# OpenGVLab/VisionLLM

Hardware: NVIDIA H100
Metric: img_text_pairs_per_sec_fwd_1024px_256tok (higher is better)
Workload: dtype bf16

## Files before the change

### include/vllm_b200.h

```cpp
#ifndef VLLM_B200_H
#define VLLM_B200_H
#include <stdint.h>
#include <stddef.h>
#ifdef __cplusplus
extern "C" {
#endif

#define VLLM_OK 0
#define VLLM_EINVAL (-1)
#define VLLM_EUNSUPPORTED (-2)
#define VLLM_EALIGN (-3)

const char* vllm_version(void);

#define VLLM_MSDA_STRICT 1
int vllm_msda_forward_f32(const float* value, const int64_t* spatial_shapes, const int64_t* level_start_index,
                          const float* sampling_loc, const float* attn_weight, float* out, int batch,
                          int spatial_size, int num_heads, int channels, int num_levels, int num_query,
                          int num_point, const int64_t* host_shapes_hint, int flags, void* stream);
int vllm_msda_forward_bf16v(const void* value, const int64_t* spatial_shapes, const int64_t* level_start_index,
                            const float* sampling_loc, const float* attn_weight, void* out, int out_bf16, int batch,
                            int spatial_size, int num_heads, int channels, int num_levels, int num_query,
                            int num_point, const int64_t* host_shapes_hint, void* stream);
int vllm_msda_forward_f64(const double* value, const int64_t* spatial_shapes, const int64_t* level_start_index,
// ... 4 lines not shown
                           const float* sampling_loc, const float* attn_weight, const float* grad_output,
                           float* grad_value, float* grad_sampling_loc, float* grad_attn_weight, int batch,
                           int spatial_size, int num_heads, int channels, int num_levels, int num_query,
                           int num_point, void* stream);
int vllm_msda_backward_f64(const double* value, const int64_t* spatial_shapes, const int64_t* level_start_index,
                           const double* sampling_loc, const double* attn_weight, const double* grad_output,
                           double* grad_value, double* grad_sampling_loc, double* grad_attn_weight, int batch,
                           int spatial_size, int num_heads, int channels, int num_levels, int num_query,
                           int num_point, void* stream);
int vllm_msda_sample_indices_f32(const int64_t* spatial_shapes, const float* sampling_loc, int32_t* out_hwm,
                                 long long n_samples, int num_levels, int num_point, void* stream);
#define VLLM_MSDA_DEFAULT 0
#define VLLM_MSDA_NO_HINT 4
#define VLLM_MSDA_BF16_NO_WINDOW 32
#define VLLM_MSDA_FP32_WINDOW 33
int vllm_msda_set_variant(int variant);
int vllm_msda_set_window(int patch_h, int patch_w, int halo0);
int vllm_msda_set_window_fill(int tma);
int vllm_msda_forward_fused_bf16(const void* value, const int64_t* level_start_index, const void* qp, int ld_qp,
                                 const float* reference_points, void* out, int out_bf16, void* attn_weights_out, int batch,
                                 int spatial_size, int num_heads, int channels, int num_levels, int num_query, int num_point,
                                 const int64_t* host_shapes_hint, void* stream);

int vllm_dcnv3_forward_f32(const float* input, const float* offset, const float* mask, float* out, int N,
                           int H_in, int W_in, int H_out, int W_out, int group, int group_channels,
                           int kernel_h, int kernel_w, int stride_h, int stride_w, int pad_h, int pad_w,
                           int dilation_h, int dilation_w, float offset_scale, int flags, void* stream);

int vllm_dcnv3_backward_f32(const float* input, const float* offset, const float* mask, const float* grad_output,
                            float* grad_input, float* grad_offset, float* grad_mask, int N, int H_in, int W_in,
                            int H_out, int W_out, int group, int group_channels, int kernel_h, int kernel_w,
                            int stride_h, int stride_w, int pad_h, int pad_w, int dilation_h, int dilation_w,
                            float offset_scale, void* stream);

#define VLLM_ACT_NONE 0
#define VLLM_ACT_GELU 1
#define VLLM_ACT_RELU 2
#define VLLM_ACT_SILU 3
#define VLLM_ACT_SWIGLU 4
#define VLLM_ACT_QUICKGELU 5
int vllm_gemm_bf16(const void* A, int lda, const void* B, int ldb, void* C, int ldc, int M, int N, int K,
                   const void* bias, const void* colscale, const void* residual, int ldr, int act, int out_f32,
                   void* stream);
int vllm_gemm_bf16_rowmask(const void* A, int lda, const void* B, int ldb, void* C, int ldc, int M, int N, int K,
                           const void* bias, const void* colscale, const void* residual, int ldr, int act, int out_f32,
                           const unsigned char* row_keep, void* stream);
int vllm_gemm_set_sm_limit(int all_gemms, int scatter_gemm);
int vllm_conv_rows_bf16(const void* xpad, long long pad_pixels, int channels, int padded_width, int kernel_h,
                        int kernel_w, const void* weight, int ldw, void* out, int ldo, int out_channels,
                        const void* bias, int act, void* stream);
#define VLLM_GEMM_DEFAULT 0
#define VLLM_GEMM_WIDE_TILE 2
#define VLLM_GEMM_NARROW_TILE 3
int vllm_gemm_set_variant(int variant);

int vllm_rmsnorm_bf16(const void* x, long long ldx, const void* weight, void* y, long long ldy, long long rows,
                      int cols, float eps, void* stream);
int vllm_layernorm_bf16(const void* x, long long ldx, const void* weight, const void* bias, void* y, long long ldy,
                        long long rows, int cols, float eps, void* stream);
int vllm_layernorm_gelu_bf16(const void* x, long long ldx, const void* weight, const void* bias, void* y,
                             long long ldy, long long rows, int cols, float eps, void* stream);
int vllm_layernorm_gather_bf16(const void* x, long long ldx, const int64_t* index, long long rows_in, long long rows_out,
                               long long batch, const void* weight, const void* bias, void* y, long long ldy, int cols,
                               float eps, void* stream);
int vllm_layernorm_residual_bf16(const void* x, long long ldx, const void* weight, const void* bias,
                                 const void* residual, long long ldr, void* y, long long ldy, long long rows, int cols,
                                 float eps, void* stream);
int vllm_dcnv3_prep_f32(const void* packed, long long ld, void* offset, void* mask, void* scale, long long rows,
                        int group, int taps, void* stream);
int vllm_dcnv3_blend_bf16(const void* core, const void* xproj, const void* scale, void* out, long long rows,
                          int channels, int group_channels, void* stream);
int vllm_dwconv_nhwc_bf16(const void* x, const void* weight_taps, const void* bias, void* y, int batch, int height,
                          int width, int channels, int kernel, void* stream);
long long vllm_groupnorm_workspace_bytes(int batch, int groups);
int vllm_groupnorm_nhwc_bf16_grid(const void* x, void* y, const void* gamma, const void* beta, int batch, long long h, long long w,
                                  long long x_w_pitch, long long x_image_pitch, int channels, int groups, float eps, int relu,
                                  void* workspace, long long workspace_bytes, void* stream);
int vllm_upsample_add_nhwc_bf16_ex(const void* top, long long top_image_pitch, const void* lateral, void* out, int batch, int in_h,
                                   int in_w, int out_h, int out_w, int channels, int out_pad, void* stream);
int vllm_rope_bf16(void* x, long long ld, const void* cos, const void* sin, long long tokens, int heads,
                   int head_dim, void* stream);

int vllm_attention_bf16(const void* q, const void* k, const void* v, void* o, int batch, int Tq, int Tk,
                        int heads, int kv_heads, int head_dim, long long q_batch_pitch,
                        long long q_token_pitch, long long k_batch_pitch, long long k_token_pitch,
                        long long v_batch_pitch, long long v_token_pitch, long long o_batch_pitch,
                        long long o_token_pitch, const int* seqlens, const unsigned char* key_mask,
                        const unsigned char* attn_mask, const float* attn_bias, int bias_batches, int causal,
                        float scale, void* workspace, long long workspace_bytes, void* stream);
int vllm_attention_mask_tiles(const unsigned char* attn_mask, long long n_batch_heads, int Tq, int Tk, int* tile_counts,
                              int* tile_lists, void* stream);
int vllm_attention_bf16_tiles(const void* q, const void* k, const void* v, void* o, int batch, int Tq, int Tk,
                              int heads, int kv_heads, int head_dim, long long q_batch_pitch,
                              long long q_token_pitch, long long k_batch_pitch, long long k_token_pitch,
                              long long v_batch_pitch, long long v_token_pitch, long long o_batch_pitch,
                              long long o_token_pitch, const int* seqlens, const unsigned char* key_mask,
                              const unsigned char* attn_mask, float scale, const int* tile_counts,
                              const int* tile_lists, void* stream);
#define VLLM_ATTN_DEFAULT 0
#define VLLM_ATTN_WARP_MMA 1
int vllm_attention_set_variant(int variant);
int vllm_attention_set_splits(int n);

int vllm_peer_alloc(void** ptr, size_t bytes);
int vllm_peer_free(void* ptr);
int vllm_peer_handle_bytes(void);
// ... 69 lines not shown
```

### visionllm_b200/_lib.py

```python
import contextlib
import ctypes
import os
import threading

_HERE = os.path.dirname(os.path.abspath(__file__))
LIB_PATH = os.path.join(_HERE, "lib", "libvllm_b200.so")

_lock = threading.Lock()
_lib = None
_launches = 0

c_i64p = ctypes.POINTER(ctypes.c_int64)
vp = ctypes.c_void_p
ci = ctypes.c_int
cll = ctypes.c_longlong
cf = ctypes.c_float

_SIGNATURES = {
    "vllm_version": (ctypes.c_char_p, []),
    "vllm_msda_forward_f32": (ci, [vp, vp, vp, vp, vp, vp, ci, ci, ci, ci, ci, ci, ci, vp, ci, vp]),
    "vllm_msda_forward_bf16v": (ci, [vp, vp, vp, vp, vp, vp, ci, ci, ci, ci, ci, ci, ci, ci, vp, vp]),
    "vllm_msda_forward_f64": (ci, [vp, vp, vp, vp, vp, vp, ci, ci, ci, ci, ci, ci, ci, vp]),
    "vllm_msda_backward_f32": (ci, [vp] * 9 + [ci] * 7 + [vp]),
    "vllm_msda_backward_f64": (ci, [vp] * 9 + [ci] * 7 + [vp]),
# ... 14 lines not shown
    "vllm_dcnv3_backward_f32": (ci, [vp] * 7 + [ci] * 15 + [cf, vp]),
    "vllm_gemm_set_sm_limit": (ci, [ci, ci]),
    "vllm_gemm_bf16": (ci, [vp, ci, vp, ci, vp, ci, ci, ci, ci, vp, vp, vp, ci, ci, ci, vp]),
    "vllm_gemm_bf16_rowmask": (ci, [vp, ci, vp, ci, vp, ci, ci, ci, ci, vp, vp, vp, ci, ci, ci, vp, vp]),
    "vllm_conv_rows_bf16": (ci, [vp, cll, ci, ci, ci, ci, vp, ci, vp, ci, ci, vp, ci, vp]),
    "vllm_gemm_bf16_tn": (ci, [vp, ci, ci, vp, ci, ci, vp, ci, ci, ci, ci, ci, vp]),
    "vllm_gemm_bf16_batched": (ci, [vp, ci, ci, vp, ci, ci, vp, ci, ci, ci, ci, ci, ci, ci, vp]),
    "vllm_gemm_bf16_batched_grouped": (ci, [vp, ci, ci, vp, ci, ci, vp, ci, ci, ci, ci, ci, ci, ci, ci, ci, vp]),
    "vllm_head_stack_bf16": (ci, [vp, vp, ci, ci, ci, ci, ci, ci, vp]),
    "vllm_head_stack_qkv_bf16": (ci, [vp, cll, vp, vp, vp, ci, ci, ci, ci, ci, ci, vp]),
    "vllm_rmsnorm_bwd_partials": (ci, [cll]),
    "vllm_rmsnorm_bwd_ws_bf16": (ci, [vp, cll, vp, vp, cll, vp, cll, vp, vp, ci, cll, ci, cf, vp]),
    "vllm_swiglu_fwd_bf16": (ci, [vp, cll, vp, cll, cll, ci, vp]),
    "vllm_swiglu_bwd_bf16": (ci, [vp, cll, vp, cll, vp, cll, cll, ci, vp]),
    "vllm_softmax_causal_bf16": (ci, [vp, cll, cll, ci, cf, vp]),
    "vllm_attn_ds_bf16": (ci, [vp, vp, cll, cll, ci, cf, vp]),
    "vllm_ce_loss_f32": (ci, [vp, cll, vp, vp, cll, ci, vp, vp, cll, vp]),
    "vllm_scale_rows_bf16": (ci, [vp, cll, cll, ci, vp, vp]),
    "vllm_gemm_set_variant": (ci, [ci]),
    "vllm_rmsnorm_bf16": (ci, [vp, cll, vp, vp, cll, cll, ci, cf, vp]),
    "vllm_layernorm_bf16": (ci, [vp, cll, vp, vp, vp, cll, cll, ci, cf, vp]),
    "vllm_layernorm_gelu_bf16": (ci, [vp, cll, vp, vp, vp, cll, cll, ci, cf, vp]),
    "vllm_layernorm_gather_bf16": (ci, [vp, cll, vp, cll, cll, cll, vp, vp, vp, cll, ci, cf, vp]),
    "vllm_layernorm_residual_bf16": (ci, [vp, cll, vp, vp, vp, cll, vp, cll, cll, ci, cf, vp]),
    "vllm_dcnv3_prep_f32": (ci, [vp, cll, vp, vp, vp, cll, ci, ci, vp]),
    "vllm_dcnv3_blend_bf16": (ci, [vp, vp, vp, vp, cll, ci, ci, vp]),
    "vllm_dwconv_nhwc_bf16": (ci, [vp, vp, vp, vp, ci, ci, ci, ci, ci, vp]),
    "vllm_rope_bf16": (ci, [vp, cll, vp, vp, cll, ci, ci, vp]),
    "vllm_groupnorm_workspace_bytes": (cll, [ci, ci]),
    "vllm_upsample_add_nhwc_bf16_ex": (ci, [vp, cll, vp, vp, ci, ci, ci, ci, ci, ci, ci, vp]),
    "vllm_groupnorm_nhwc_bf16_grid": (ci, [vp, vp, vp, vp, ci, cll, cll, cll, cll, ci, ci, cf, ci, vp, cll, vp]),
    "vllm_attention_bf16": (ci, [vp, vp, vp, vp, ci, ci, ci, ci, ci, ci, cll, cll, cll, cll, cll, cll, cll, cll,
                                 vp, vp, vp, vp, ci, ci, cf, vp, cll, vp]),
    "vllm_attention_bf16_tiles": (ci, [vp, vp, vp, vp, ci, ci, ci, ci, ci, ci, cll, cll, cll, cll, cll, cll, cll, cll,
                                       vp, vp, vp, cf, vp, vp, vp]),
    "vllm_attention_mask_tiles": (ci, [vp, cll, ci, ci, vp, vp, vp]),
    "vllm_attention_set_variant": (ci, [ci]),
    "vllm_attention_set_splits": (ci, [ci]),
    "vllm_peer_alloc": (ci, [ctypes.POINTER(vp), ctypes.c_size_t]),
    "vllm_peer_free": (ci, [vp]),
    "vllm_peer_handle_bytes": (ci, []),
    "vllm_peer_export": (ci, [vp, vp]),
    "vllm_peer_open": (ci, [vp, ctypes.POINTER(vp)]),
    "vllm_peer_close": (ci, [vp]),
    "vllm_gemm_bf16_scatter": (ci, [vp, ci, vp, ci, vp, vp, ci, ci, ci, ci, ci, vp]),
    "vllm_tp_reduce_norm_bf16": (ci, [vp, ci, cll, vp, vp, cf, vp, ci, cll, vp, ctypes.c_uint, vp, ci, ci, ci, vp]),
    "vllm_tp_norm_ctas": (ci, [ci]),
    "vllm_tp_wait": (ci, [vp, ctypes.c_uint, vp]),
    "vllm_tp_signal": (ci, [vp, ci, ctypes.c_uint, vp]),
}


MSDA_DEFAULT, MSDA_NO_HINT, MSDA_BF16_NO_WINDOW, MSDA_FP32_WINDOW = 0, 4, 32, 33
GEMM_DEFAULT, GEMM_WIDE_TILE, GEMM_NARROW_TILE = 0, 2, 3
ATTN_DEFAULT, ATTN_WARP_MMA = 0, 1

_KNOB_DEFAULTS = {"msda_set_variant": (MSDA_DEFAULT,), "msda_set_window": (0, 0, 0), "msda_set_window_fill": (-1,),
                  "gemm_set_variant": (GEMM_DEFAULT,), "gemm_set_sm_limit": (0, 0), "attention_set_variant": (ATTN_DEFAULT,),
                  "attention_set_splits": (0,)}


class VllmB200Error(RuntimeError):
    pass


def exported_symbols():
    return sorted(_SIGNATURES)


def lib():
    global _lib
    if _lib is None:
        with _lock:
            if _lib is None:
                if not os.path.exists(LIB_PATH):
                    raise ImportError(
                        f"{LIB_PATH} is missing: build it with `make` or "
                        "`python -c 'import __graft_entry__ as g; g.build()'`. "
                        "visionllm_b200 has no CPU/eager fallback.")
                L = ctypes.CDLL(LIB_PATH)
                for name, (res, args) in _SIGNATURES.items():
                    fn = getattr(L, name)
                    fn.restype = res
                    fn.argtypes = args
                _lib = L
    return _lib


_ERR = {-1: "invalid argument", -2: "unsupported shape", -3: "misaligned pointer"}


def check(rc, what):
    global _launches
    _launches += 1
    if rc == 0:
        return
    if rc < 0:
        raise VllmB200Error(f"{what}: {_ERR.get(rc, 'error')} (rc={rc})")
    raise VllmB200Error(f"{what}: CUDA error {rc} at launch")


@contextlib.contextmanager
def knob(name, *values):
    fn = getattr(lib(), "vllm_" + name)
    rc = fn(*values)
    if rc != 0:
        raise VllmB200Error(f"vllm_{name}{values}: {_ERR.get(rc, 'error')} (rc={rc})")
# ... 14 lines not shown
```

### visionllm_b200/csrc/gemm.cu

```cuda
#include "common.cuh"
#include "tc_common.cuh"
#include "vllm_b200.h"

namespace {

constexpr int BM = 128, BK = 64, THREADS = 384, CONSUMER_WARPS = 8, CONSUMER_THREADS = CONSUMER_WARPS * 32;
constexpr int A_BYTES = BM * BK * 2;
constexpr int EPI_BUF = 16 * 128;
constexpr int SMEM_LIMIT = 232448;

enum { ACT_NONE = 0, ACT_GELU = 1, ACT_RELU = 2, ACT_SILU = 3, ACT_SWIGLU = 4, ACT_QUICKGELU = 5 };

struct GemmArgs {
  int M, N, K;
  void* C; int ldc;
  const __nv_bfloat16* bias; const __nv_bfloat16* colscale; const __nv_bfloat16* residual; int ldr;
  int act; int out_f32;
  const unsigned char* row_keep;
  int tiles_m, tiles_n;
  int group_m;
  int a_seg_kb, a_seg_rows;
  int sc_rows;
  void* sc_dst[8];
  uint32_t* sc_flag[8];
  int a_mn, b_mn;
  int bt_rows, causal;
  int group, reduce;
};

struct TilePlan { int skip, kb0, kb1, segs, b_row_off, a_k_off, b_k_off; };
__device__ __forceinline__ TilePlan plan_tile(const GemmArgs& g, int m0, int n0, int rows_per_tile, int num_kb) {
  TilePlan p{0, 0, num_kb, 1, 0, 0, 0};
  if (g.bt_rows) {
    const int bh = m0 / g.bt_rows, ml = m0 - bh * g.bt_rows;
    const int a_mat = g.reduce ? bh * g.group : bh;
    const int b_mat = g.reduce ? bh * g.group : bh / g.group;
    p.segs = g.reduce ? g.group : 1;
    p.b_row_off = b_mat * g.N;
    p.a_k_off = a_mat * g.K;
    p.b_k_off = b_mat * g.K;
    if (g.causal == 1 && n0 >= ml + rows_per_tile) p.skip = 1;
    if (g.causal == 2) p.kb0 = ml / BK;
    if (g.causal == 3) { const int e = (ml + rows_per_tile + BK - 1) / BK; p.kb1 = e < num_kb ? e : num_kb; }
  }
  return p;
}

template <int BN> struct Cfg {
  static constexpr int B_BYTES = BN * BK * 2;
  static constexpr int STAGE_BYTES = A_BYTES + B_BYTES;
  static constexpr int STAGES = BN == 256 ? 4 : 6;
  static constexpr int EPI_OFF = STAGES * STAGE_BYTES;
  static constexpr int BAR_OFF = EPI_OFF + CONSUMER_WARPS * 2 * EPI_BUF;
  static constexpr int BIAS_OFF = BAR_OFF + 256;
  static constexpr int SCALE_OFF = BIAS_OFF + 2 * BN + 4;
  static constexpr int KEEP_OFF = SCALE_OFF + 2 * BN + 4;
  static constexpr int SMEM = 1024  + KEEP_OFF + BM + 4;
  static_assert(8 * (2 * STAGES + 2 * CONSUMER_WARPS) <= 256, "mbarriers overflow their slot");
  static_assert(SMEM <= SMEM_LIMIT, "shared memory over the per-block limit");
};

__device__ __forceinline__ float gelu_erf(float x) { return 0.5f * x * (1.f + erff(x * 0.70710678118654752f)); }
__device__ __forceinline__ float silu(float x) { return x / (1.f + __expf(-x)); }

__device__ __forceinline__ void tile_coords(int t, int tiles_m, int tiles_n, int group_m, int& tm, int& tn) {
  const int per_group = group_m * tiles_n;
  const int group = t / per_group;
  const int first = group * group_m;
  const int gsz = min(group_m, tiles_m - first);
  const int in = t - group * per_group;
  tm = first + in % gsz;
  tn = in / gsz;
}

template <int BN, int TA, int TB>
__device__ __forceinline__ void mma_kblock(float (&acc)[BN / 2], uint32_t sa, uint32_t sb, bool first_kb) {
  const uint64_t adesc = TA ? tc::wgmma_desc_sw128(sa, 8192, 1024) : tc::wgmma_desc_sw128(sa, 16, 1024);
  const uint64_t bdesc = TB ? tc::wgmma_desc_sw128(sb, 8192, 1024) : tc::wgmma_desc_sw128(sb, 16, 1024);
  constexpr uint64_t astep = TA ? 128 : 2, bstep = TB ? 128 : 2;
#pragma unroll
  for (int k = 0; k < BK / 16; ++k) {
    if constexpr (BN == 256)
      tc::wgmma_m64n256k16_ss<TA, TB>(acc, adesc + astep * k, bdesc + bstep * k, !(first_kb && k == 0));
    else
      tc::wgmma_m64n128k16_ss<TA, TB>(acc, adesc + astep * k, bdesc + bstep * k, !(first_kb && k == 0));
  }
}

enum { EPI_BF16 = 0, EPI_SWIGLU = 1, EPI_F32 = 2, EPI_SCATTER = 3 };

__device__ __forceinline__ int swz(int r, int b) { return r * 128 + ((((b >> 4) ^ r) & 7) << 4) + (b & 15); }

template <int BN, int TA, int TB, int EPI>
__global__ void __launch_bounds__(THREADS, 1)
gemm_bf16_wgmma_kernel(const __grid_constant__ CUtensorMap tmap_a, const __grid_constant__ CUtensorMap tmap_b,
                       const __grid_constant__ CUtensorMap tmap_c, const __grid_constant__ CUtensorMap tmap_r,
                       const GemmArgs g) {
  using C_ = Cfg<BN>;
  constexpr int STAGES = C_::STAGES;
  extern __shared__ uint8_t smem_raw[];
  const uint32_t smem_base = (tc::smem_u32(smem_raw) + 1023u) & ~1023u;
  uint8_t* smem_gen = smem_raw + (smem_base - tc::smem_u32(smem_raw));
  const uint32_t bar_base = smem_base + C_::BAR_OFF;
  auto full_bar = [&](int s) { return bar_base + 8 * s; };
  auto empty_bar = [&](int s) { return bar_base + 8 * (STAGES + s); };
  auto res_bar = [&](int i) { return bar_base + 8 * (2 * STAGES + i); };

  const int warp = threadIdx.x >> 5, lane = threadIdx.x & 31;
  const int n_tiles = g.tiles_m * g.tiles_n;
  const int num_kb = (g.K + BK - 1) / BK;

  if (warp == 0 && lane == 0) {
    tc::tma_prefetch_desc(&tmap_a);
    tc::tma_prefetch_desc(&tmap_b);
    if constexpr (EPI != EPI_SCATTER) {
      tc::tma_prefetch_desc(&tmap_c);
      if (g.residual) tc::tma_prefetch_desc(&tmap_r);
    }
  }
  if (warp == 1 && lane == 0) {
    for (int s = 0; s < STAGES; ++s) { tc::mbar_init(full_bar(s), 1); tc::mbar_init(empty_bar(s), CONSUMER_WARPS); }
    for (int i = 0; i < 2 * CONSUMER_WARPS; ++i) tc::mbar_init(res_bar(i), 1);
    tc::mbar_fence_init();
  }
  __syncthreads();

  if (warp < 4) {
    tc::reg_dealloc<40>();
    if (warp == 0 && tc::elect_one()) {
      int stage = 0; uint32_t phase = 0;
      for (int t = blockIdx.x; t < n_tiles; t += gridDim.x) {
        int tm, tn; tile_coords(t, g.tiles_m, g.tiles_n, g.group_m, tm, tn);
        const TilePlan tp = plan_tile(g, tm * BM, tn * BN, BM, num_kb);
        if (tp.skip) continue;
        const int bt_m0 = g.bt_rows ? (tm * BM) / g.bt_rows * g.bt_rows : 0;
        const int row_a = tm * BM - (TA ? bt_m0 : 0);
        const int row_b = tn * BN + (TB ? 0 : tp.b_row_off);
        for (int gs = 0; gs < tp.segs; ++gs) {
          const int ka_off = TA ? tp.a_k_off + gs * g.K : 0, kb_off = TB ? tp.b_k_off + gs * g.K : 0;
          for (int kb = tp.kb0; kb < tp.kb1; ++kb) {
            tc::mbar_wait(empty_bar(stage), phase ^ 1);
            const uint32_t sa = smem_base + stage * C_::STAGE_BYTES, sb = sa + A_BYTES;
            int ka = kb * BK + ka_off, ra = row_a;
            if (g.a_seg_kb) {
              const int seg = kb / g.a_seg_kb;
              ka = (kb - seg * g.a_seg_kb) * BK;
              ra = row_a + seg * g.a_seg_rows;
            }
            tc::mbar_arrive_expect_tx(full_bar(stage), C_::STAGE_BYTES);
            if constexpr (TA) {
              for (int h = 0; h < BM / 64; ++h) tc::tma_load_2d(sa + h * 8192, &tmap_a, full_bar(stage), ra + 64 * h, ka);
            } else {
              tc::tma_load_2d(sa, &tmap_a, full_bar(stage), ka, ra);
            }
            if constexpr (TB) {
              for (int h = 0; h < BN / 64; ++h)
                tc::tma_load_2d(sb + h * 8192, &tmap_b, full_bar(stage), row_b + 64 * h, kb * BK + kb_off);
            } else {
              tc::tma_load_2d(sb, &tmap_b, full_bar(stage), kb * BK, row_b);
            }
            if (++stage == STAGES) { stage = 0; phase ^= 1; }
          }
        }
      }
    }
    return;
  }

  tc::reg_alloc<232>();
  const int wg = (warp - 4) >> 2;
  const int cw = warp - 4;
  const int et = threadIdx.x - 128;
  const int lr = lane >> 2, frag_col = 2 * (lane & 3);
  const bool has_res = EPI != EPI_SCATTER && g.residual != nullptr;
  constexpr int UNIT_COLS = EPI == EPI_SWIGLU ? 128 : 64;
  constexpr int UNITS = BN / UNIT_COLS;
  constexpr int RES_AHEAD = EPI == EPI_F32 ? 1 : 2;
  const int n_out = EPI == EPI_SWIGLU ? g.N / 2 : g.N;
  uint8_t* s_buf = smem_gen + C_::EPI_OFF + cw * 2 * EPI_BUF;
  const uint32_t s_buf_u32 = smem_base + C_::EPI_OFF + cw * 2 * EPI_BUF;
  const uint32_t s_bias = smem_base + C_::BIAS_OFF, s_scale = smem_base + C_::SCALE_OFF, s_keep = smem_base + C_::KEEP_OFF;
  const __nv_bfloat16* bias_t = reinterpret_cast<const __nv_bfloat16*>(smem_gen + C_::BIAS_OFF + (reinterpret_cast<uintptr_t>(g.bias) & 3));
  const __nv_bfloat16* scale_t =
      reinterpret_cast<const __nv_bfloat16*>(smem_gen + C_::SCALE_OFF + (reinterpret_cast<uintptr_t>(g.colscale) & 3));
  const uint8_t* keep_t = smem_gen + C_::KEEP_OFF + (reinterpret_cast<uintptr_t>(g.row_keep) & 3);
  if (et <= BN / 2) {
    if (!g.bias) *reinterpret_cast<uint32_t*>(smem_gen + C_::BIAS_OFF + 4 * et) = 0u;
    if (!g.colscale) *reinterpret_cast<uint32_t*>(smem_gen + C_::SCALE_OFF + 4 * et) = 0x3F803F80u;
  }
  uint32_t res_phase = 0;
  int stage = 0; uint32_t phase = 0;
  float acc[BN / 2];
  for (int t = blockIdx.x; t < n_tiles; t += gridDim.x) {
    int tm, tn; tile_coords(t, g.tiles_m, g.tiles_n, g.group_m, tm, tn);
    const TilePlan tp = plan_tile(g, tm * BM, tn * BN, BM, num_kb);
    if (tp.skip) continue;
    const int n0 = tn * BN;
    const int oc0 = EPI == EPI_SWIGLU ? n0 / 2 : n0;
    const int warp_row0 = tm * BM + cw * 16;
    const bool warp_live = warp_row0 < g.M;
    if (g.bias && et <= BN / 2) tc::cp_async_vec_word(s_bias, g.bias, 2LL * g.N, 2LL * n0, et);
    if (g.colscale && et <= BN / 2) tc::cp_async_vec_word(s_scale, g.colscale, 2LL * g.N, 2LL * n0, et);
    if (g.row_keep && et <= BM / 4) tc::cp_async_vec_word(s_keep, g.row_keep, g.M, (long long)tm * BM, et);
    auto load_res = [&](int u) {
      const int b = EPI == EPI_F32 ? 0 : (u & 1);
      tc::mbar_arrive_expect_tx(res_bar(2 * cw + b), EPI_BUF);
      tc::tma_load_2d(s_buf_u32 + b * EPI_BUF, &tmap_r, res_bar(2 * cw + b), oc0 + 64 * u, warp_row0);
    };
    if (has_res && warp_live && lane == 0) {
      tc::bulk_wait_read<0>();
#pragma unroll
      for (int u = 0; u < RES_AHEAD && u < UNITS; ++u)
        if (oc0 + 64 * u < n_out) load_res(u);
    }
    int prev_stage = -1;
    const int n_kb = tp.segs * (tp.kb1 - tp.kb0);
    for (int kb = 0; kb < n_kb; ++kb) {
      tc::mbar_wait(full_bar(stage), phase);
      const uint32_t sa = smem_base + stage * C_::STAGE_BYTES + wg * 8192, sb = smem_base + stage * C_::STAGE_BYTES + A_BYTES;
      const bool first = kb == 0;
      tc::acc_fence(acc);
      tc::wgmma_fence();
      mma_kblock<BN, TA, TB>(acc, sa, sb, first);
      tc::wgmma_commit();
      tc::wgmma_wait<1>();
      if (prev_stage >= 0 && lane == 0) tc::mbar_arrive(empty_bar(prev_stage));
      prev_stage = stage;
      if (++stage == STAGES) { stage = 0; phase ^= 1; }
    }
    tc::wgmma_wait<0>();
    tc::acc_fence(acc);
    if (lane == 0) tc::mbar_arrive(empty_bar(prev_stage));
    tc::cp_async_wait_all();
    tc::named_bar_sync(1, CONSUMER_THREADS);

#pragma unroll
    for (int j = 0; j < BN / 8; ++j) {
      const int c = 8 * j + frag_col;
      const float b0 = __bfloat162float(bias_t[c]), b1 = __bfloat162float(bias_t[c + 1]);
      acc[4 * j] = __fadd_rn(acc[4 * j], b0); acc[4 * j + 1] = __fadd_rn(acc[4 * j + 1], b1);
      acc[4 * j + 2] = __fadd_rn(acc[4 * j + 2], b0); acc[4 * j + 3] = __fadd_rn(acc[4 * j + 3], b1);
    }
    if constexpr (EPI == EPI_BF16 || EPI == EPI_F32) {
      switch (g.act) {
        case ACT_GELU:
#pragma unroll
          for (int i = 0; i < BN / 2; ++i) acc[i] = gelu_erf(acc[i]);
          break;
        case ACT_RELU:
#pragma unroll
          for (int i = 0; i < BN / 2; ++i) acc[i] = fmaxf(acc[i], 0.f);
          break;
        case ACT_SILU:
#pragma unroll
          for (int i = 0; i < BN / 2; ++i) acc[i] = silu(acc[i]);
          break;
        case ACT_QUICKGELU:
#pragma unroll
          for (int i = 0; i < BN / 2; ++i) acc[i] = acc[i] / (1.f + __expf(-1.702f * acc[i]));
          break;
        default: break;
      }
    }
    bool keep0 = true, keep1 = true;
    if (g.row_keep) { keep0 = keep_t[cw * 16 + lr] != 0; keep1 = keep_t[cw * 16 + lr + 8] != 0; }

    constexpr int E = EPI == EPI_F32 ? 4 : 2;
    auto put_box = [&](int bi, int col0) {
      if ((n_out * E) % 16 == 0 || col0 + 128 / E <= n_out) {
        if (lane == 0) tc::tma_store_2d(&tmap_c, s_buf_u32 + bi * EPI_BUF, col0, warp_row0);
        return;
      }
#pragma unroll
      for (int it = 0; it < 4; ++it) {
        const int rr = it * 4 + (lane >> 3), piece = lane & 7, row = warp_row0 + rr;
        if (row >= g.M) continue;
#pragma unroll
        for (int e = 0; e < 16 / E; ++e) {
          const int col = col0 + piece * (16 / E) + e;
          if (col >= n_out) break;
          const uint8_t* sp = s_buf + bi * EPI_BUF + swz(rr, 16 * piece + E * e);
          uint8_t* dp = reinterpret_cast<uint8_t*>(g.C) + ((size_t)row * g.ldc + col) * E;
          if constexpr (E == 4) *reinterpret_cast<uint32_t*>(dp) = *reinterpret_cast<const uint32_t*>(sp);
          else *reinterpret_cast<uint16_t*>(dp) = *reinterpret_cast<const uint16_t*>(sp);
        }
      }
    };

    if (warp_live) {
#pragma unroll
      for (int u = 0; u < UNITS; ++u) {
        if (oc0 + 64 * u >= n_out) break;
        const int b = EPI == EPI_F32 ? 0 : (u & 1);
        uint8_t* buf = s_buf + b * EPI_BUF;
        if (has_res) {
          if (u > 0 && u + RES_AHEAD - 1 < UNITS && oc0 + 64 * (u + RES_AHEAD - 1) < n_out && lane == 0) {
            tc::bulk_wait_read<0>();
            load_res(u + RES_AHEAD - 1);
          }
          tc::mbar_wait(res_bar(2 * cw + b), (res_phase >> b) & 1);
          res_phase ^= 1u << b;
        } else if constexpr (EPI != EPI_SCATTER && EPI != EPI_F32) {
          if (lane == 0) { if (u == 0) tc::bulk_wait_read<0>(); else tc::bulk_wait_read<1>(); }
          __syncwarp();
        }
        if constexpr (EPI == EPI_SWIGLU) {
#pragma unroll
          for (int jj = 0; jj < 16; ++jj) {
            const int j = 16 * u + jj;
#pragma unroll
            for (int h = 0; h < 2; ++h) {
              uint8_t* p = buf + swz(lr + 8 * h, 16 * (jj >> 1)) + 8 * (jj & 1) + 2 * (lane & 3);
              float o = __fmul_rn(silu(acc[4 * j + 2 * h]), acc[4 * j + 2 * h + 1]);
              if (has_res) o = __fadd_rn(o, __bfloat162float(*reinterpret_cast<const __nv_bfloat16*>(p)));
              *reinterpret_cast<__nv_bfloat16*>(p) = __float2bfloat16(o);
            }
          }
        } else {
// ... 9 lines not shown
              v0 = __fmul_rn(v0, s0); v1 = __fmul_rn(v1, s1);
              if (has_res) {
                const float2 f = __bfloat1622float2(*reinterpret_cast<const __nv_bfloat162*>(p));
                v0 = __fadd_rn(v0, f.x); v1 = __fadd_rn(v1, f.y);
              }
              if (!(h ? keep1 : keep0)) { v0 = 0.f; v1 = 0.f; }
              if constexpr (EPI != EPI_F32) *reinterpret_cast<__nv_bfloat162*>(p) = __floats2bfloat162_rn(v0, v1);
            }
          }
          if constexpr (EPI == EPI_F32) {
            if (lane == 0) tc::bulk_wait_read<0>();
            __syncwarp();
#pragma unroll
            for (int jj = 0; jj < 8; ++jj) {
              const int j = 8 * u + jj;
#pragma unroll
              for (int h = 0; h < 2; ++h) {
                uint8_t* p = s_buf + (jj >> 2) * EPI_BUF + swz(lr + 8 * h, 32 * (jj & 3) + 8 * (lane & 3));
                *reinterpret_cast<float2*>(p) = make_float2(acc[4 * j + 2 * h], acc[4 * j + 2 * h + 1]);
              }
            }
          }
        }
        if constexpr (EPI == EPI_SCATTER) {
          __syncwarp();
          const int d = warp_row0 / g.sc_rows;
          __nv_bfloat16* dst = reinterpret_cast<__nv_bfloat16*>(g.sc_dst[d]) + (size_t)(warp_row0 - d * g.sc_rows) * g.ldc + n0 + 64 * u;
#pragma unroll
          for (int it = 0; it < 4; ++it) {
            const int rr = it * 4 + (lane >> 3), piece = lane & 7;
            const uint4 val = *reinterpret_cast<const uint4*>(buf + swz(rr, 16 * piece));
            *reinterpret_cast<uint4*>(dst + (size_t)rr * g.ldc + piece * 8) = val;
          }
          __syncwarp();
        } else {
          tc::fence_proxy_async_smem();
          __syncwarp();
          if constexpr (EPI == EPI_F32) {
            put_box(0, n0 + 64 * u);
            if (n0 + 64 * u + 32 < n_out) put_box(1, n0 + 64 * u + 32);
          } else {
            put_box(b, oc0 + 64 * u);
          }
          if (lane == 0) tc::bulk_commit();
        }
      }
    }
    if constexpr (EPI == EPI_SCATTER) {
      __threadfence_system();
      __syncwarp();
      if (lane == 0 && warp_live)
        asm volatile("red.release.sys.global.add.u32 [%0], %1;" ::"l"(g.sc_flag[warp_row0 / g.sc_rows]), "r"(1u) : "memory");
    }
    tc::named_bar_sync(1, CONSUMER_THREADS);
  }
  if (EPI != EPI_SCATTER && lane == 0) tc::bulk_wait<0>();
}

int g_sm_limit = 0, g_scatter_sm_limit = 0;

int g_gemm_variant = VLLM_GEMM_DEFAULT;

using KernelFn = void (*)(const CUtensorMap, const CUtensorMap, const CUtensorMap, const CUtensorMap, const GemmArgs);

template <int BN, int TA, int TB>
KernelFn pick_epilogue(const GemmArgs& g) {
  if (g.sc_rows) {
    if constexpr (BN == 256 && !TA && !TB) return gemm_bf16_wgmma_kernel<BN, TA, TB, EPI_SCATTER>;
    return nullptr;
  }
  if (g.act == ACT_SWIGLU) {
    if constexpr (!TA && !TB) return gemm_bf16_wgmma_kernel<BN, TA, TB, EPI_SWIGLU>;
    return nullptr;
  }
  if (g.out_f32) return gemm_bf16_wgmma_kernel<BN, TA, TB, EPI_F32>;
  return gemm_bf16_wgmma_kernel<BN, TA, TB, EPI_BF16>;
}
template <int BN>
KernelFn pick_kernel(const GemmArgs& g) {
  if (g.a_mn) return g.b_mn ? pick_epilogue<BN, 1, 1>(g) : pick_epilogue<BN, 1, 0>(g);
  return g.b_mn ? pick_epilogue<BN, 0, 1>(g) : pick_epilogue<BN, 0, 0>(g);
}

template <int BN>
int launch_gemm(const void* A, int lda, const void* B, int ldb, GemmArgs g, cudaStream_t st, long long a_rows = -1,
                int a_cols = -1) {
  using C_ = Cfg<BN>;
  CUtensorMap ta, tb;
  const uint64_t nb = g.bt_rows ? (uint64_t)(g.M / g.bt_rows) : 1;
  const uint64_t na = g.bt_rows && g.reduce ? nb * g.group : nb;
  const uint64_t nbb = !g.bt_rows ? 1 : g.reduce ? nb * g.group : nb / g.group;
  const uint64_t m_local = g.bt_rows ? (uint64_t)g.bt_rows : (uint64_t)g.M;
  int rc = g.a_mn ? vllm_make_tmap_2d(&ta, A, na * (uint64_t)g.K, m_local, (uint64_t)lda, 64)
                  : vllm_make_tmap_2d(&ta, A, (uint64_t)(a_rows < 0 ? g.M : a_rows),
                                        (uint64_t)(a_cols < 0 ? g.K : a_cols), (uint64_t)lda, BM);
  if (rc) return rc;
  rc = g.b_mn ? vllm_make_tmap_2d(&tb, B, nbb * (uint64_t)g.K, (uint64_t)g.N, (uint64_t)ldb, 64)
              : vllm_make_tmap_2d(&tb, B, nbb * (uint64_t)g.N, (uint64_t)g.K, (uint64_t)ldb, BN);
  if (rc) return rc;
  CUtensorMap tc_{}, tr{};
  if (!g.sc_rows) {
    const uint64_t n_out = (uint64_t)(g.act == ACT_SWIGLU ? g.N / 2 : g.N);
    rc = vllm_make_tmap_2d(&tc_, g.C, (uint64_t)g.M, n_out, (uint64_t)g.ldc, 16, g.out_f32 != 0);
    if (!rc && g.residual) rc = vllm_make_tmap_2d(&tr, g.residual, (uint64_t)g.M, n_out, (uint64_t)g.ldr, 16);
    if (rc) return rc;
  }
  g.tiles_m = (g.M + BM - 1) / BM;
  g.tiles_n = (g.N + BN - 1) / BN;
  const int n_tiles = g.tiles_m * g.tiles_n;
  int sms = vllm_num_sms();
  const int limit = g.sc_rows ? (g_scatter_sm_limit > 0 ? g_scatter_sm_limit : g_sm_limit) : g_sm_limit;
  if (limit > 0 && limit < sms) sms = limit;
  const int ctas = sms < n_tiles ? sms : n_tiles;
  g.group_m = 8;
  const KernelFn kern = pick_kernel<BN>(g);
  if (!kern) return VLLM_EUNSUPPORTED;
  const cudaError_t e = vllm_smem_optin(kern, C_::SMEM);
  if (e != cudaSuccess) return (int)e;
  kern<<<ctas, THREADS, C_::SMEM, st>>>(ta, tb, tc_, tr, g);
  VLLM_CHECK_LAUNCH();
  return VLLM_OK;
}

bool wide_by_shape(const GemmArgs& g) {
  return !g.a_mn && !g.b_mn && !g.bt_rows && !g.a_seg_kb && g.N >= 2048;
}

int launch_gemm_auto(const void* A, int lda, const void* B, int ldb, const GemmArgs& g, cudaStream_t st, long long a_rows = -1,
                     int a_cols = -1) {
  const bool wide = g.sc_rows || g_gemm_variant == VLLM_GEMM_WIDE_TILE ||
                    (g_gemm_variant == VLLM_GEMM_DEFAULT && wide_by_shape(g));
  return wide ? launch_gemm<256>(A, lda, B, ldb, g, st, a_rows, a_cols) : launch_gemm<128>(A, lda, B, ldb, g, st, a_rows, a_cols);
}

}

extern "C" {

int vllm_gemm_set_variant(int v) {
  if (v != VLLM_GEMM_DEFAULT && v != VLLM_GEMM_WIDE_TILE && v != VLLM_GEMM_NARROW_TILE) return VLLM_EINVAL;
  g_gemm_variant = v;
  return VLLM_OK;
}
int vllm_gemm_set_sm_limit(int all_gemms, int scatter_gemm) {
  if (all_gemms < 0 || scatter_gemm < 0) return VLLM_EINVAL;
  g_sm_limit = all_gemms; g_scatter_sm_limit = scatter_gemm;
  return VLLM_OK;
}

static int gemm_bf16_common(const void* A, int lda, const void* B, int ldb, void* C, int ldc, int M, int N, int K,
                            const void* bias, const void* colscale, const void* residual, int ldr, int act, int out_f32,
                            const unsigned char* row_keep, void* stream);

int vllm_gemm_bf16(const void* A, int lda, const void* B, int ldb, void* C, int ldc, int M, int N, int K,
                   const void* bias, const void* colscale, const void* residual, int ldr, int act, int out_f32,
                   void* stream) {
  return gemm_bf16_common(A, lda, B, ldb, C, ldc, M, N, K, bias, colscale, residual, ldr, act, out_f32, nullptr, stream);
}

int vllm_gemm_bf16_rowmask(const void* A, int lda, const void* B, int ldb, void* C, int ldc, int M, int N, int K,
                           const void* bias, const void* colscale, const void* residual, int ldr, int act, int out_f32,
                           const unsigned char* row_keep, void* stream) {
  if (!row_keep || act == ACT_SWIGLU) return VLLM_EINVAL;
  return gemm_bf16_common(A, lda, B, ldb, C, ldc, M, N, K, bias, colscale, residual, ldr, act, out_f32, row_keep, stream);
}

static int gemm_bf16_common(const void* A, int lda, const void* B, int ldb, void* C, int ldc, int M, int N, int K,
                            const void* bias, const void* colscale, const void* residual, int ldr, int act, int out_f32,
                            const unsigned char* row_keep, void* stream) {
  if (M < 0 || N <= 0 || K <= 0 || lda < K || ldb < K) return VLLM_EINVAL;
  if (M == 0) return VLLM_OK;
  if (!A || !B || !C) return VLLM_EINVAL;
  if (act < 0 || act > ACT_QUICKGELU) return VLLM_EINVAL;
  const int n_out = act == ACT_SWIGLU ? N / 2 : N;
  if (act == ACT_SWIGLU && (N % 2 || out_f32 || colscale)) return VLLM_EUNSUPPORTED;
  if (ldc < n_out || (residual && ldr < n_out)) return VLLM_EINVAL;
  if (!vllm_aligned(A, 16) || !vllm_aligned(B, 16) || (lda % 8) || (ldb % 8)) return VLLM_EALIGN;
  const int celt = out_f32 ? 4 : 2;
  if (!vllm_aligned(C, 16) || ((size_t)ldc * celt) % 16 || (residual && (!vllm_aligned(residual, 16) || ldr % 8)))
    return VLLM_EALIGN;
  GemmArgs g{};
  g.M = M; g.N = N; g.K = K; g.C = C; g.ldc = ldc;
  g.bias = (const __nv_bfloat16*)bias; g.colscale = (const __nv_bfloat16*)colscale;
  g.residual = (const __nv_bfloat16*)residual; g.ldr = ldr; g.act = act; g.out_f32 = out_f32;
  g.row_keep = row_keep;
  cudaStream_t st = (cudaStream_t)stream;
  return launch_gemm_auto(A, lda, B, ldb, g, st);
}

int vllm_gemm_bf16_tn(const void* A, int lda, int a_mn_major, const void* B, int ldb, int b_mn_major, void* C, int ldc, int M,
                      int N, int K, int out_f32, void* stream) {
  if (M < 0 || N <= 0 || K <= 0) return VLLM_EINVAL;
  if (M == 0) return VLLM_OK;
// ... 84 lines not shown
```

Before: 7.065.

## Add ping-pong warpgroup GEMM variant for GELU/SwiGLU epilogue GEMMs

Adds a ping-pong persistent GEMM schedule in which the two consumer warpgroups each own alternate 64x256 tiles. A turn barrier orders their mainloops so one warpgroup's epilogue overlaps the other's MMA mainloop. It is enabled by default for dense K-major GEMMs with GELU or SwiGLU activation, where the heavy epilogue was meant to be hidden. The tradeoff is smaller M tiles, which mean more B reloads per output, plus a duplicated per-warpgroup bias/scale buffer and extra barriers.

```diff
diff --git a/include/vllm_b200.h b/include/vllm_b200.h
--- a/include/vllm_b200.h
+++ b/include/vllm_b200.h
@@ -80,6 +80,7 @@
 #define VLLM_GEMM_DEFAULT 0
 #define VLLM_GEMM_WIDE_TILE 2
 #define VLLM_GEMM_NARROW_TILE 3
+#define VLLM_GEMM_PINGPONG 4
 int vllm_gemm_set_variant(int variant);
 
 int vllm_rmsnorm_bf16(const void* x, long long ldx, const void* weight, void* y, long long ldy, long long rows,
diff --git a/visionllm_b200/_lib.py b/visionllm_b200/_lib.py
--- a/visionllm_b200/_lib.py
+++ b/visionllm_b200/_lib.py
@@ -90,7 +90,7 @@
 
 
 MSDA_DEFAULT, MSDA_NO_HINT, MSDA_BF16_NO_WINDOW, MSDA_FP32_WINDOW = 0, 4, 32, 33
-GEMM_DEFAULT, GEMM_WIDE_TILE, GEMM_NARROW_TILE = 0, 2, 3
+GEMM_DEFAULT, GEMM_WIDE_TILE, GEMM_NARROW_TILE, GEMM_PINGPONG = 0, 2, 3, 4
 ATTN_DEFAULT, ATTN_WARP_MMA = 0, 1
 
 _KNOB_DEFAULTS = {"msda_set_variant": (MSDA_DEFAULT,), "msda_set_window": (0, 0, 0), "msda_set_window_fill": (-1,),
diff --git a/visionllm_b200/csrc/gemm.cu b/visionllm_b200/csrc/gemm.cu
--- a/visionllm_b200/csrc/gemm.cu
+++ b/visionllm_b200/csrc/gemm.cu
@@ -5,7 +5,6 @@
 namespace {
 
 constexpr int BM = 128, BK = 64, THREADS = 384, CONSUMER_WARPS = 8, CONSUMER_THREADS = CONSUMER_WARPS * 32;
-constexpr int A_BYTES = BM * BK * 2;
 constexpr int EPI_BUF = 16 * 128;
 constexpr int SMEM_LIMIT = 232448;
 
@@ -46,17 +45,21 @@
   return p;
 }
 
-template <int BN> struct Cfg {
+template <int BN, int PP = 0> struct Cfg {
   static constexpr int B_BYTES = BN * BK * 2;
-  static constexpr int STAGE_BYTES = A_BYTES + B_BYTES;
+  static constexpr int TM = PP ? 64 : BM;
+  static constexpr int A_TILE = TM * BK * 2;
+  static constexpr int STAGE_BYTES = A_TILE + B_BYTES;
   static constexpr int STAGES = BN == 256 ? 4 : 6;
   static constexpr int EPI_OFF = STAGES * STAGE_BYTES;
   static constexpr int BAR_OFF = EPI_OFF + CONSUMER_WARPS * 2 * EPI_BUF;
   static constexpr int BIAS_OFF = BAR_OFF + 256;
   static constexpr int SCALE_OFF = BIAS_OFF + 2 * BN + 4;
   static constexpr int KEEP_OFF = SCALE_OFF + 2 * BN + 4;
-  static constexpr int SMEM = 1024  + KEEP_OFF + BM + 4;
-  static_assert(8 * (2 * STAGES + 2 * CONSUMER_WARPS) <= 256, "mbarriers overflow their slot");
+  static constexpr int VEC_BYTES = KEEP_OFF + BM + 4 - BIAS_OFF;
+  static constexpr int SMEM = 1024  + BIAS_OFF + (PP ? 2 : 1) * VEC_BYTES;
+  static_assert(VEC_BYTES % 4 == 0, "vector sets must stay word-aligned");
+  static_assert(8 * (2 * STAGES + 2 * CONSUMER_WARPS + 2) <= 256, "mbarriers overflow their slot");
   static_assert(SMEM <= SMEM_LIMIT, "shared memory over the per-block limit");
 };
 
@@ -91,12 +94,13 @@
 
 __device__ __forceinline__ int swz(int r, int b) { return r * 128 + ((((b >> 4) ^ r) & 7) << 4) + (b & 15); }
 
-template <int BN, int TA, int TB, int EPI>
+template <int BN, int TA, int TB, int EPI, int PP = 0>
 __global__ void __launch_bounds__(THREADS, 1)
 gemm_bf16_wgmma_kernel(const __grid_constant__ CUtensorMap tmap_a, const __grid_constant__ CUtensorMap tmap_b,
                        const __grid_constant__ CUtensorMap tmap_c, const __grid_constant__ CUtensorMap tmap_r,
                        const GemmArgs g) {
-  using C_ = Cfg<BN>;
+  static_assert(!PP || (BN == 256 && !TA && !TB && EPI != EPI_SCATTER), "ping-pong: dense K-major 64 x 256 tiles only");
+  using C_ = Cfg<BN, PP>;
   constexpr int STAGES = C_::STAGES;
   extern __shared__ uint8_t smem_raw[];
   const uint32_t smem_base = (tc::smem_u32(smem_raw) + 1023u) & ~1023u;
@@ -105,6 +109,7 @@
   auto full_bar = [&](int s) { return bar_base + 8 * s; };
   auto empty_bar = [&](int s) { return bar_base + 8 * (STAGES + s); };
   auto res_bar = [&](int i) { return bar_base + 8 * (2 * STAGES + i); };
+  auto turn_bar = [&](int w) { return bar_base + 8 * (2 * STAGES + 2 * CONSUMER_WARPS + w); };
 
   const int warp = threadIdx.x >> 5, lane = threadIdx.x & 31;
   const int n_tiles = g.tiles_m * g.tiles_n;
@@ -119,8 +124,9 @@
     }
   }
   if (warp == 1 && lane == 0) {
-    for (int s = 0; s < STAGES; ++s) { tc::mbar_init(full_bar(s), 1); tc::mbar_init(empty_bar(s), CONSUMER_WARPS); }
+    for (int s = 0; s < STAGES; ++s) { tc::mbar_init(full_bar(s), 1); tc::mbar_init(empty_bar(s), PP ? 4 : CONSUMER_WARPS); }
     for (int i = 0; i < 2 * CONSUMER_WARPS; ++i) tc::mbar_init(res_bar(i), 1);
+    if (PP) { tc::mbar_init(turn_bar(0), 4); tc::mbar_init(turn_bar(1), 4); }
     tc::mbar_fence_init();
   }
   __syncthreads();
@@ -131,16 +137,16 @@
       int stage = 0; uint32_t phase = 0;
       for (int t = blockIdx.x; t < n_tiles; t += gridDim.x) {
         int tm, tn; tile_coords(t, g.tiles_m, g.tiles_n, g.group_m, tm, tn);
-        const TilePlan tp = plan_tile(g, tm * BM, tn * BN, BM, num_kb);
+        const TilePlan tp = plan_tile(g, tm * C_::TM, tn * BN, C_::TM, num_kb);
         if (tp.skip) continue;
         const int bt_m0 = g.bt_rows ? (tm * BM) / g.bt_rows * g.bt_rows : 0;
-        const int row_a = tm * BM - (TA ? bt_m0 : 0);
+        const int row_a = tm * C_::TM - (TA ? bt_m0 : 0);
         const int row_b = tn * BN + (TB ? 0 : tp.b_row_off);
         for (int gs = 0; gs < tp.segs; ++gs) {
           const int ka_off = TA ? tp.a_k_off + gs * g.K : 0, kb_off = TB ? tp.b_k_off + gs * g.K : 0;
           for (int kb = tp.kb0; kb < tp.kb1; ++kb) {
             tc::mbar_wait(empty_bar(stage), phase ^ 1);
-            const uint32_t sa = smem_base + stage * C_::STAGE_BYTES, sb = sa + A_BYTES;
+            const uint32_t sa = smem_base + stage * C_::STAGE_BYTES, sb = sa + C_::A_TILE;
             int ka = kb * BK + ka_off, ra = row_a;
             if (g.a_seg_kb) {
               const int seg = kb / g.a_seg_kb;
@@ -168,9 +174,14 @@
   }
 
   tc::reg_alloc<232>();
+  constexpr int TM = C_::TM;
+  constexpr int SYNC_THREADS = PP ? 128 : CONSUMER_THREADS;
   const int wg = (warp - 4) >> 2;
   const int cw = warp - 4;
   const int et = threadIdx.x - 128;
+  const int vt = PP ? et & 127 : et;
+  const int sync_id = PP ? 1 + wg : 1;
+  const int warp_row = PP ? 16 * (cw & 3) : 16 * cw;
   const int lr = lane >> 2, frag_col = 2 * (lane & 3);
   const bool has_res = EPI != EPI_SCATTER && g.residual != nullptr;
   constexpr int UNIT_COLS = EPI == EPI_SWIGLU ? 128 : 64;
@@ -179,29 +190,40 @@
   const int n_out = EPI == EPI_SWIGLU ? g.N / 2 : g.N;
   uint8_t* s_buf = smem_gen + C_::EPI_OFF + cw * 2 * EPI_BUF;
   const uint32_t s_buf_u32 = smem_base + C_::EPI_OFF + cw * 2 * EPI_BUF;
-  const uint32_t s_bias = smem_base + C_::BIAS_OFF, s_scale = smem_base + C_::SCALE_OFF, s_keep = smem_base + C_::KEEP_OFF;
-  const __nv_bfloat16* bias_t = reinterpret_cast<const __nv_bfloat16*>(smem_gen + C_::BIAS_OFF + (reinterpret_cast<uintptr_t>(g.bias) & 3));
+  const int vec_off = PP ? wg * C_::VEC_BYTES : 0;
+  const uint32_t s_bias = smem_base + C_::BIAS_OFF + vec_off, s_scale = smem_base + C_::SCALE_OFF + vec_off,
+                 s_keep = smem_base + C_::KEEP_OFF + vec_off;
+  const __nv_bfloat16* bias_t =
+      reinterpret_cast<const __nv_bfloat16*>(smem_gen + C_::BIAS_OFF + vec_off + (reinterpret_cast<uintptr_t>(g.bias) & 3));
   const __nv_bfloat16* scale_t =
-      reinterpret_cast<const __nv_bfloat16*>(smem_gen + C_::SCALE_OFF + (reinterpret_cast<uintptr_t>(g.colscale) & 3));
-  const uint8_t* keep_t = smem_gen + C_::KEEP_OFF + (reinterpret_cast<uintptr_t>(g.row_keep) & 3);
-  if (et <= BN / 2) {
-    if (!g.bias) *reinterpret_cast<uint32_t*>(smem_gen + C_::BIAS_OFF + 4 * et) = 0u;
-    if (!g.colscale) *reinterpret_cast<uint32_t*>(smem_gen + C_::SCALE_OFF + 4 * et) = 0x3F803F80u;
+      reinterpret_cast<const __nv_bfloat16*>(smem_gen + C_::SCALE_OFF + vec_off + (reinterpret_cast<uintptr_t>(g.colscale) & 3));
+  const uint8_t* keep_t = smem_gen + C_::KEEP_OFF + vec_off + (reinterpret_cast<uintptr_t>(g.row_keep) & 3);
+  if (vt <= BN / 2) {
+    if (!g.bias) *reinterpret_cast<uint32_t*>(smem_gen + C_::BIAS_OFF + vec_off + 4 * vt) = 0u;
+    if (!g.colscale) *reinterpret_cast<uint32_t*>(smem_gen + C_::SCALE_OFF + vec_off + 4 * vt) = 0x3F803F80u;
   }
   uint32_t res_phase = 0;
+  uint32_t turn_phase = 0;
   int stage = 0; uint32_t phase = 0;
   float acc[BN / 2];
-  for (int t = blockIdx.x; t < n_tiles; t += gridDim.x) {
+  for (int t = blockIdx.x, seq = 0; t < n_tiles; t += gridDim.x, ++seq) {
     int tm, tn; tile_coords(t, g.tiles_m, g.tiles_n, g.group_m, tm, tn);
-    const TilePlan tp = plan_tile(g, tm * BM, tn * BN, BM, num_kb);
+    const TilePlan tp = plan_tile(g, tm * TM, tn * BN, TM, num_kb);
     if (tp.skip) continue;
+    const int n_kb = tp.segs * (tp.kb1 - tp.kb0);
+    if (PP && (seq & 1) != wg) {
+      stage += n_kb;
+      phase ^= (stage / STAGES) & 1;
+      stage %= STAGES;
+      continue;
+    }
     const int n0 = tn * BN;
     const int oc0 = EPI == EPI_SWIGLU ? n0 / 2 : n0;
-    const int warp_row0 = tm * BM + cw * 16;
+    const int warp_row0 = tm * TM + warp_row;
     const bool warp_live = warp_row0 < g.M;
-    if (g.bias && et <= BN / 2) tc::cp_async_vec_word(s_bias, g.bias, 2LL * g.N, 2LL * n0, et);
-    if (g.colscale && et <= BN / 2) tc::cp_async_vec_word(s_scale, g.colscale, 2LL * g.N, 2LL * n0, et);
-    if (g.row_keep && et <= BM / 4) tc::cp_async_vec_word(s_keep, g.row_keep, g.M, (long long)tm * BM, et);
+    if (g.bias && vt <= BN / 2) tc::cp_async_vec_word(s_bias, g.bias, 2LL * g.N, 2LL * n0, vt);
+    if (g.colscale && vt <= BN / 2) tc::cp_async_vec_word(s_scale, g.colscale, 2LL * g.N, 2LL * n0, vt);
+    if (g.row_keep && vt <= TM / 4) tc::cp_async_vec_word(s_keep, g.row_keep, g.M, (long long)tm * TM, vt);
     auto load_res = [&](int u) {
       const int b = EPI == EPI_F32 ? 0 : (u & 1);
       tc::mbar_arrive_expect_tx(res_bar(2 * cw + b), EPI_BUF);
@@ -213,11 +235,15 @@
       for (int u = 0; u < RES_AHEAD && u < UNITS; ++u)
         if (oc0 + 64 * u < n_out) load_res(u);
     }
+    if (PP && seq > 0) {
+      tc::mbar_wait(turn_bar(wg), turn_phase);
+      turn_phase ^= 1;
+    }
     int prev_stage = -1;
-    const int n_kb = tp.segs * (tp.kb1 - tp.kb0);
     for (int kb = 0; kb < n_kb; ++kb) {
       tc::mbar_wait(full_bar(stage), phase);
-      const uint32_t sa = smem_base + stage * C_::STAGE_BYTES + wg * 8192, sb = smem_base + stage * C_::STAGE_BYTES + A_BYTES;
+      const uint32_t sa = smem_base + stage * C_::STAGE_BYTES + (PP ? 0 : wg * 8192);
+      const uint32_t sb = smem_base + stage * C_::STAGE_BYTES + C_::A_TILE;
       const bool first = kb == 0;
       tc::acc_fence(acc);
       tc::wgmma_fence();
@@ -228,11 +254,12 @@
       prev_stage = stage;
       if (++stage == STAGES) { stage = 0; phase ^= 1; }
     }
+    if (PP && t + gridDim.x < n_tiles && lane == 0) tc::mbar_arrive(turn_bar(wg ^ 1));
     tc::wgmma_wait<0>();
     tc::acc_fence(acc);
     if (lane == 0) tc::mbar_arrive(empty_bar(prev_stage));
     tc::cp_async_wait_all();
-    tc::named_bar_sync(1, CONSUMER_THREADS);
+    tc::named_bar_sync(sync_id, SYNC_THREADS);
 
 #pragma unroll
     for (int j = 0; j < BN / 8; ++j) {
@@ -263,7 +290,7 @@
       }
     }
     bool keep0 = true, keep1 = true;
-    if (g.row_keep) { keep0 = keep_t[cw * 16 + lr] != 0; keep1 = keep_t[cw * 16 + lr + 8] != 0; }
+    if (g.row_keep) { keep0 = keep_t[warp_row + lr] != 0; keep1 = keep_t[warp_row + lr + 8] != 0; }
 
     constexpr int E = EPI == EPI_F32 ? 4 : 2;
     auto put_box = [&](int bi, int col0) {
@@ -379,7 +406,7 @@
       if (lane == 0 && warp_live)
         asm volatile("red.release.sys.global.add.u32 [%0], %1;" ::"l"(g.sc_flag[warp_row0 / g.sc_rows]), "r"(1u) : "memory");
     }
-    tc::named_bar_sync(1, CONSUMER_THREADS);
+    tc::named_bar_sync(sync_id, SYNC_THREADS);
   }
   if (EPI != EPI_SCATTER && lane == 0) tc::bulk_wait<0>();
 }
@@ -390,8 +417,13 @@
 
 using KernelFn = void (*)(const CUtensorMap, const CUtensorMap, const CUtensorMap, const CUtensorMap, const GemmArgs);
 
-template <int BN, int TA, int TB>
+template <int BN, int TA, int TB, int PP>
 KernelFn pick_epilogue(const GemmArgs& g) {
+  if constexpr (PP) {
+    if (g.act == ACT_SWIGLU) return gemm_bf16_wgmma_kernel<BN, 0, 0, EPI_SWIGLU, 1>;
+    if (g.out_f32) return gemm_bf16_wgmma_kernel<BN, 0, 0, EPI_F32, 1>;
+    return gemm_bf16_wgmma_kernel<BN, 0, 0, EPI_BF16, 1>;
+  }
   if (g.sc_rows) {
     if constexpr (BN == 256 && !TA && !TB) return gemm_bf16_wgmma_kernel<BN, TA, TB, EPI_SCATTER>;
     return nullptr;
@@ -403,16 +435,17 @@
   if (g.out_f32) return gemm_bf16_wgmma_kernel<BN, TA, TB, EPI_F32>;
   return gemm_bf16_wgmma_kernel<BN, TA, TB, EPI_BF16>;
 }
-template <int BN>
+template <int BN, int PP>
 KernelFn pick_kernel(const GemmArgs& g) {
-  if (g.a_mn) return g.b_mn ? pick_epilogue<BN, 1, 1>(g) : pick_epilogue<BN, 1, 0>(g);
-  return g.b_mn ? pick_epilogue<BN, 0, 1>(g) : pick_epilogue<BN, 0, 0>(g);
-}
-
-template <int BN>
+  if constexpr (PP) return pick_epilogue<BN, 0, 0, 1>(g);
+  if (g.a_mn) return g.b_mn ? pick_epilogue<BN, 1, 1, 0>(g) : pick_epilogue<BN, 1, 0, 0>(g);
+  return g.b_mn ? pick_epilogue<BN, 0, 1, 0>(g) : pick_epilogue<BN, 0, 0, 0>(g);
+}
+
+template <int BN, int PP = 0>
 int launch_gemm(const void* A, int lda, const void* B, int ldb, GemmArgs g, cudaStream_t st, long long a_rows = -1,
                 int a_cols = -1) {
-  using C_ = Cfg<BN>;
+  using C_ = Cfg<BN, PP>;
   CUtensorMap ta, tb;
   const uint64_t nb = g.bt_rows ? (uint64_t)(g.M / g.bt_rows) : 1;
   const uint64_t na = g.bt_rows && g.reduce ? nb * g.group : nb;
@@ -420,7 +453,7 @@
   const uint64_t m_local = g.bt_rows ? (uint64_t)g.bt_rows : (uint64_t)g.M;
   int rc = g.a_mn ? vllm_make_tmap_2d(&ta, A, na * (uint64_t)g.K, m_local, (uint64_t)lda, 64)
                   : vllm_make_tmap_2d(&ta, A, (uint64_t)(a_rows < 0 ? g.M : a_rows),
-                                        (uint64_t)(a_cols < 0 ? g.K : a_cols), (uint64_t)lda, BM);
+                                        (uint64_t)(a_cols < 0 ? g.K : a_cols), (uint64_t)lda, C_::TM);
   if (rc) return rc;
   rc = g.b_mn ? vllm_make_tmap_2d(&tb, B, nbb * (uint64_t)g.K, (uint64_t)g.N, (uint64_t)ldb, 64)
               : vllm_make_tmap_2d(&tb, B, nbb * (uint64_t)g.N, (uint64_t)g.K, (uint64_t)ldb, BN);
@@ -432,15 +465,15 @@
     if (!rc && g.residual) rc = vllm_make_tmap_2d(&tr, g.residual, (uint64_t)g.M, n_out, (uint64_t)g.ldr, 16);
     if (rc) return rc;
   }
-  g.tiles_m = (g.M + BM - 1) / BM;
+  g.tiles_m = (g.M + C_::TM - 1) / C_::TM;
   g.tiles_n = (g.N + BN - 1) / BN;
   const int n_tiles = g.tiles_m * g.tiles_n;
   int sms = vllm_num_sms();
   const int limit = g.sc_rows ? (g_scatter_sm_limit > 0 ? g_scatter_sm_limit : g_sm_limit) : g_sm_limit;
   if (limit > 0 && limit < sms) sms = limit;
   const int ctas = sms < n_tiles ? sms : n_tiles;
-  g.group_m = 8;
-  const KernelFn kern = pick_kernel<BN>(g);
+  g.group_m = 8 * BM / C_::TM;
+  const KernelFn kern = pick_kernel<BN, PP>(g);
   if (!kern) return VLLM_EUNSUPPORTED;
   const cudaError_t e = vllm_smem_optin(kern, C_::SMEM);
   if (e != cudaSuccess) return (int)e;
@@ -453,8 +486,19 @@
   return !g.a_mn && !g.b_mn && !g.bt_rows && !g.a_seg_kb && g.N >= 2048;
 }
 
+bool pingpong_ok(const GemmArgs& g) {
+  return !g.a_mn && !g.b_mn && !g.bt_rows && !g.a_seg_kb && !g.sc_rows;
+}
+
+bool pingpong_by_shape(const GemmArgs& g) {
+  return pingpong_ok(g) && (g.act == ACT_GELU || g.act == ACT_SWIGLU);
+}
+
 int launch_gemm_auto(const void* A, int lda, const void* B, int ldb, const GemmArgs& g, cudaStream_t st, long long a_rows = -1,
                      int a_cols = -1) {
+  if ((g_gemm_variant == VLLM_GEMM_PINGPONG && pingpong_ok(g)) ||
+      (g_gemm_variant == VLLM_GEMM_DEFAULT && pingpong_by_shape(g)))
+    return launch_gemm<256, 1>(A, lda, B, ldb, g, st, a_rows, a_cols);
   const bool wide = g.sc_rows || g_gemm_variant == VLLM_GEMM_WIDE_TILE ||
                     (g_gemm_variant == VLLM_GEMM_DEFAULT && wide_by_shape(g));
   return wide ? launch_gemm<256>(A, lda, B, ldb, g, st, a_rows, a_cols) : launch_gemm<128>(A, lda, B, ldb, g, st, a_rows, a_cols);
@@ -465,7 +509,8 @@
 extern "C" {
 
 int vllm_gemm_set_variant(int v) {
-  if (v != VLLM_GEMM_DEFAULT && v != VLLM_GEMM_WIDE_TILE && v != VLLM_GEMM_NARROW_TILE) return VLLM_EINVAL;
+  if (v != VLLM_GEMM_DEFAULT && v != VLLM_GEMM_WIDE_TILE && v != VLLM_GEMM_NARROW_TILE && v != VLLM_GEMM_PINGPONG)
+    return VLLM_EINVAL;
   g_gemm_variant = v;
   return VLLM_OK;
 }
```

Result: faster. 7.228, median of 6 (+2.3%).
